# ofsoundof/GRL-Image-Restoration

Measured on NVIDIA H100. Metric: Mpix/s (input pixels) GRL-Base x4 SR 256x256 tiles, higher is better.
Workload: dtype f16

## Files before the change

### grl-image-restoration_b200/csrc/gemm_tc.cu

```cuda
#include <algorithm>

#include "grl_common.cuh"
#include "tc_common.cuh"
#include "ops_tc.h"

namespace grl {
namespace tc {

EncodeTiledFn encode_tiled_fn() {
  static EncodeTiledFn fn = nullptr;
  if (!fn) {
    void* p = nullptr;
    cudaDriverEntryPointQueryResult q;
    if (cudaGetDriverEntryPoint("cuTensorMapEncodeTiled", &p, cudaEnableDefault, &q) == cudaSuccess &&
        q == cudaDriverEntryPointSuccess)
      fn = (EncodeTiledFn)p;
  }
  return fn;
}

__device__ __forceinline__ float gelu_as(float x) {
  const float z = fabsf(x) * 0.70710678118654752440f;
  float t, e;
  asm("rcp.approx.ftz.f32 %0, %1;" : "=f"(t) : "f"(fmaf(0.3275911f, z, 1.0f)));
  asm("ex2.approx.ftz.f32 %0, %1;" : "=f"(e) : "f"(-z * z * 1.4426950408889634f));
  float p = fmaf(1.061405429f, t, -1.453152027f);
  p = fmaf(p, t, 1.421413741f);
  p = fmaf(p, t, -0.284496736f);
  p = fmaf(p, t, 0.254829592f);
  const float erf_abs = fmaf(-p * t, e, 1.0f);
  const float half_x = 0.5f * x;
  return fmaf(half_x, copysignf(erf_abs, x), half_x);
}
__device__ __forceinline__ float tc_act(float v, int act, float slope) {
  if (act == GRL_ACT_GELU) return gelu_as(v);
  if (act == GRL_ACT_LEAKY) return v > 0.f ? v : v * slope;
  return v;
}

constexpr int kStages = 4;
constexpr int kBM = 128, kBK = 64;
constexpr int kTH = 8, kTW = 16;
constexpr int kEpiWarps = 8, kEpiThreads = kEpiWarps * 32, kThreads = kEpiThreads + 32;

__host__ __device__ constexpr int stage_pitch32(int c) { return (c % 8 == 4) ? c : ((c + 3) / 4 * 4 % 8 == 4 ? (c + 3) / 4 * 4 : (c + 3) / 4 * 4 + 4); }

template <int BN>
struct GemmSmem {
  static constexpr int A_BYTES = kBM * kBK * 2;
  static constexpr int B_BYTES = BN * kBK * 2;
  static constexpr int STAGE = A_BYTES + B_BYTES;
  static constexpr int PIPE = kStages * STAGE;
  static constexpr int AP = BN + 4;
  static constexpr int ACC = kBM * AP * 4;
  static constexpr int STG32 = kBM * stage_pitch32(BN <= 192 ? (BN == 192 ? 188 : BN) : 4) * 4;
  static constexpr int STG16 = kBM * (BN + 8) * 2;
  static constexpr int STG = (STG32 > STG16 ? STG32 : STG16);
  static constexpr int OFF_STG = ACC;
  static constexpr int OFF_TOK = ((PIPE > ACC + STG ? PIPE : ACC + STG) + 15) / 16 * 16;
  static constexpr int OFF_PAR = OFF_TOK + 128 * 8 + 128 * 4;
  static constexpr int OFF_MOM = OFF_PAR + 3 * BN * 4;
  static constexpr int OFF_BAR = OFF_MOM + 2 * 128 * 3 * 4;
  static constexpr int TOTAL = OFF_BAR + 128 + 1024 ;
  static_assert(AP % 8 == 4, "accumulator pitch");
  static_assert(TOTAL <= 232448, "shared memory budget");
};

__device__ __forceinline__ void epi_barrier() { asm volatile("bar.sync 1, 256;" ::: "memory"); }

__device__ __forceinline__ void acc_row32(const float* p, uint32_t (&v)[32]) {
#pragma unroll
  for (int j = 0; j < 32; j += 4) {
    const uint4 x = *reinterpret_cast<const uint4*>(p + j);
    v[j] = x.x, v[j + 1] = x.y, v[j + 2] = x.z, v[j + 3] = x.w;
  }
}

template <int BN, int FMT>
__device__ __forceinline__ void mma_loop(float (&acc)[BN / 64][32], uint8_t* smem, uint64_t* full, uint64_t* empty,
                                         int nk_total, int half, int et) {
  using S = GemmSmem<BN>;
  for (int kc = 0; kc < nk_total; ++kc) {
    const int s = kc % kStages;
    mbar_wait(&full[s], (kc / kStages) & 1);
    const uint32_t sa = smem_u32(smem + s * S::STAGE) + half * (64 * 128);
    const uint32_t sb = smem_u32(smem + s * S::STAGE + S::A_BYTES);
    wgmma_fence();
#pragma unroll
    for (int k = 0; k < kBK / 16; ++k) {
      const uint64_t ad = gmma_desc(sa + k * 32, 16, 1024, SWZ_128B);
#pragma unroll
      for (int j = 0; j < BN / 64; ++j) {
        const uint64_t bd = gmma_desc(sb + j * (64 * 128) + k * 32, 16, 1024, SWZ_128B);
        if (FMT == FMT_BF16) wgmma_n64_bf16(acc[j], ad, bd, true);
        else wgmma_n64_f16(acc[j], ad, bd, true);
      }
    }
    wgmma_commit();
    wgmma_wait<1>();
    if (kc > 0 && (et & 127) == 0) mbar_arrive(&empty[(kc - 1) % kStages]);
  }
  wgmma_wait<0>();
}

template <int BN, int EPI, bool CONV>
__global__ void __launch_bounds__(kThreads, 1)
gemm_tc_kernel(const __grid_constant__ CUtensorMap tmA, const __grid_constant__ CUtensorMap tmB, const GemmTcArgs a) {
  extern __shared__ uint8_t smem_raw[];
  uint8_t* smem = reinterpret_cast<uint8_t*>((reinterpret_cast<uintptr_t>(smem_raw) + 1023) & ~uintptr_t(1023));
  using S = GemmSmem<BN>;
  constexpr int AP = S::AP;
  uint64_t* full = reinterpret_cast<uint64_t*>(smem + S::OFF_BAR);
  uint64_t* empty = full + kStages;
  long long* s_tok = reinterpret_cast<long long*>(smem + S::OFF_TOK);
  int* s_img = reinterpret_cast<int*>(smem + S::OFF_TOK + 128 * 8);
  float* s_bias = reinterpret_cast<float*>(smem + S::OFF_PAR);
  float* s_gamma = s_bias + BN;
  float* s_beta = s_gamma + BN;
  float* s_mom = reinterpret_cast<float*>(smem + S::OFF_MOM);
  float* accs = reinterpret_cast<float*>(smem);

  const int warp = threadIdx.x >> 5, lane = threadIdx.x & 31;
  const int n_tiles = a.n_tiles;
  const int m_idx = blockIdx.x / n_tiles;
  const int n0 = (blockIdx.x - m_idx * n_tiles) * BN;
  const int nk_total = a.taps * a.nk;
  int m0 = 0, tb = 0, ty0 = 0, tx0 = 0;
  if (CONV) {
    int t = m_idx;
    const int tx = t % a.tiles_x;
    t /= a.tiles_x;
    const int ty = t % a.tiles_y;
    tb = t / a.tiles_y;
    ty0 = ty * kTH;
    tx0 = tx * kTW;
  } else {
    m0 = m_idx * kBM;
  }

  if (threadIdx.x == 0) {
    for (int s = 0; s < kStages; ++s) {
      mbar_init(&full[s], 1);
      mbar_init(&empty[s], 2);
    }
    mbar_init_fence();
    tma_prefetch_desc(&tmA);
    tma_prefetch_desc(&tmB);
  }
  __syncthreads();

  if (warp == kEpiWarps) {
    if (lane == 0) {
      for (int kc = 0; kc < nk_total; ++kc) {
        const int s = kc % kStages;
        mbar_wait(&empty[s], ((kc / kStages) & 1) ^ 1);
        uint8_t* sa = smem + s * S::STAGE;
        uint8_t* sb = sa + S::A_BYTES;
        mbar_expect_tx(&full[s], S::STAGE);
        if (CONV) {
          const int tap = kc / a.nk, c0 = (kc - tap * a.nk) * kBK;
          tma_load_4d(sa, &tmA, &full[s], c0, tx0 + (tap % 3) - 1, ty0 + (tap / 3) - 1, tb);
        } else {
          tma_load_2d(sa, &tmA, &full[s], kc * kBK, m0);
        }
        tma_load_2d(sb, &tmB, &full[s], kc * kBK, n0);
      }
    }
    return;
  }

  const int et = threadIdx.x;
  const int q = warp & 3;
  const int row = q * 32 + lane;
  const int half = et >> 7;
  const int fmt = a.fmt;
  uint16_t* out16 = reinterpret_cast<uint16_t*>(a.out_bf16);
  {
    long long tok;
    if (CONV) {
      const int y = ty0 + row / kTW, x = tx0 + row % kTW;
      tok = (y < a.H && x < a.W) ? ((long long)tb * a.H + y) * a.W + x : -1;
    } else {
      tok = (long long)m0 + row;
      if (tok >= a.M) tok = -1;
    }
    if (half == 0) {
      s_tok[row] = tok;
      s_img[row] = (EPI == EPI_LN && tok >= 0) ? (int)(tok / a.L) : 0;
    }
    for (int c = et; c < BN; c += kEpiThreads) {
      const int n = n0 + c;
      s_bias[c] = (n < a.N) ? a.bias[n] : 0.f;
      if (EPI == EPI_LN) {
        s_gamma[c] = (c < a.C) ? a.gamma[c] : 0.f;
        s_beta[c] = (c < a.C) ? a.beta[c] : 0.f;
      }
    }
  }
  {
    float acc[BN / 64][32];
#pragma unroll
    for (int j = 0; j < BN / 64; ++j)
#pragma unroll
      for (int e = 0; e < 32; ++e) acc[j][e] = 0.f;
    if (fmt == FMT_BF16) mma_loop<BN, FMT_BF16>(acc, smem, full, empty, nk_total, half, et);
    else mma_loop<BN, FMT_F16>(acc, smem, full, empty, nk_total, half, et);
    epi_barrier();
    const int w = (et >> 5) & 3, r0 = half * 64 + 16 * w + (lane >> 2), cq = 2 * (lane & 3);
#pragma unroll
    for (int j = 0; j < BN / 64; ++j)
#pragma unroll
      for (int i = 0; i < 8; ++i) {
        const int c = j * 64 + 8 * i + cq;
        *reinterpret_cast<float2*>(accs + r0 * AP + c) = make_float2(acc[j][4 * i], acc[j][4 * i + 1]);
        *reinterpret_cast<float2*>(accs + (r0 + 8) * AP + c) = make_float2(acc[j][4 * i + 2], acc[j][4 * i + 3]);
      }
  }
  epi_barrier();
  uint32_t v[32];

    if (EPI == EPI_BIAS_ACT && a.epi_mode == 2) {
      const long long tok = s_tok[row];
      for (int c0 = 32 * half; c0 < BN; c0 += 64) {
        if (n0 + c0 >= a.N) break;
        acc_row32(accs + row * AP + c0, v);
        if (tok < 0) continue;
        float o[32];
#pragma unroll
        for (int j = 0; j < 32; ++j) {
          const int n = n0 + c0 + j;
          float val = tc_act(__uint_as_float(v[j]) + s_bias[c0 + j], a.act, a.slope);
          if (a.res_f32 && n < a.N_f32) val += __ldg(a.res_f32 + tok * a.ldr + n);
          o[j] = (n < a.N) ? val : 0.f;
          if (a.out_f32 && n < a.N_f32) a.out_f32[tok * a.ldo_f32 + n] = o[j];
          if (CONV && a.out_nchw && n < a.N_f32) {
            const int r = a.nchw_r, rr = r * r;
            const int c = n / rr, q = n - c * rr;
            const int yy = (ty0 + row / kTW) * r + q / r, xx = (tx0 + row % kTW) * r + q % r;
            if (yy < a.Hc && xx < a.Wc)
              a.out_nchw[(((long long)tb * (a.N_f32 / rr) + c) * a.Hc + yy) * a.Wc + xx] = fmaf(o[j], a.post_scale, a.post_shift[c & 3]);
          }
        }
        if (out16) {
#pragma unroll
          for (int j = 0; j < 32; j += 8)
            if (n0 + c0 + j < a.ldo_bf16)
              *reinterpret_cast<uint4*>(out16 + tok * a.ldo_bf16 + n0 + c0 + j) =
                  make_uint4(pack16(o[j], o[j + 1], fmt), pack16(o[j + 2], o[j + 3], fmt), pack16(o[j + 4], o[j + 5], fmt),
                             pack16(o[j + 6], o[j + 7], fmt));
        }
      }
    } else if (a.epi_mode == 1) {
      const int Cw = (EPI == EPI_LN) ? a.C : a.N_f32;
      const int pitch = stage_pitch32(Cw);
      float* stg = reinterpret_cast<float*>(smem + S::OFF_STG);
      const bool res_in_stage = a.res_f32 != nullptr;
      if (res_in_stage) {
        const int C4r = Cw >> 2, ewr = et >> 5;
        for (int r = ewr; r < kBM; r += kEpiWarps) {
          const long long rtok = s_tok[r];
          for (int c4 = lane; c4 < C4r; c4 += 32)
            cp_async_16(stg + r * pitch + c4 * 4, a.res_f32 + (rtok >= 0 ? rtok : 0) * a.ldr + c4 * 4, rtok >= 0);
        }
        cp_async_commit();
      }
      if (EPI == EPI_LN) {
        float s1 = 0.f, s2 = 0.f, x0 = 0.f;
        int nh = 0;
        for (int c0 = 32 * half; c0 < Cw; c0 += 64) {
          acc_row32(accs + row * AP + c0, v);
          if (c0 == 32 * half) x0 = __uint_as_float(v[0]) + s_bias[c0];
#pragma unroll
          for (int j = 0; j < 32; ++j)
            if (c0 + j < Cw) {
              const float d = __uint_as_float(v[j]) + s_bias[c0 + j] - x0;
              s1 += d;
              s2 = fmaf(d, d, s2);
              ++nh;
            }
        }
        {
          const float fn = (float)nh;
          const float m1 = nh > 0 ? s1 / fn : 0.f;
          s_mom[(half * kBM + row) * 3 + 0] = x0 + m1;
          s_mom[(half * kBM + row) * 3 + 1] = nh > 0 ? fmaxf(s2 - s1 * m1, 0.f) : 0.f;
          s_mom[(half * kBM + row) * 3 + 2] = fn;
        }
        if (res_in_stage) cp_async_wait<0>();
        epi_barrier();
        float mean, rstd;
        {
          const float m0 = s_mom[row * 3 + 0], q0 = s_mom[row * 3 + 1], c0n = s_mom[row * 3 + 2];
          const float m1 = s_mom[(kBM + row) * 3 + 0], q1 = s_mom[(kBM + row) * 3 + 1], c1n = s_mom[(kBM + row) * 3 + 2];
          const float n = c0n + c1n, d = (c1n > 0.f) ? m1 - m0 : 0.f;
          mean = m0 + d * (c1n / n);
          const float M2 = q0 + q1 + d * d * (c0n * c1n / n);
          rstd = rsqrtf(M2 / n + a.eps);
        }
        for (int c0 = 32 * half; c0 < Cw; c0 += 64) {
          acc_row32(accs + row * AP + c0, v);
#pragma unroll
          for (int j = 0; j < 32; j += 4) {
            if (c0 + j < Cw) {
              float4* sp = reinterpret_cast<float4*>(stg + row * pitch + c0 + j);
              float4 acc4 = res_in_stage ? *sp : make_float4(0.f, 0.f, 0.f, 0.f);
              float o4[4] = {acc4.x, acc4.y, acc4.z, acc4.w};
#pragma unroll
              for (int e = 0; e < 4; ++e) {
                const int c = c0 + j + e;
                o4[e] += ((__uint_as_float(v[j + e]) + s_bias[c] - mean) * rstd * s_gamma[c] + s_beta[c]) * a.res_scale;
              }
              *sp = make_float4(o4[0], o4[1], o4[2], o4[3]);
            }
          }
        }
      } else {
        if (res_in_stage) {
          cp_async_wait<0>();
          epi_barrier();
        }
        for (int c0 = 32 * half; c0 < Cw; c0 += 64) {
          acc_row32(accs + row * AP + c0, v);
#pragma unroll
          for (int j = 0; j < 32; j += 4) {
            if (c0 + j < Cw) {
              float4* sp = reinterpret_cast<float4*>(stg + row * pitch + c0 + j);
              float4 acc4 = res_in_stage ? *sp : make_float4(0.f, 0.f, 0.f, 0.f);
              float o4[4] = {acc4.x, acc4.y, acc4.z, acc4.w};
#pragma unroll
              for (int e = 0; e < 4; ++e) o4[e] += tc_act(__uint_as_float(v[j + e]) + s_bias[c0 + j + e], a.act, a.slope);
              *sp = make_float4(o4[0], o4[1], o4[2], o4[3]);
            }
          }
        }
      }
      epi_barrier();
      const int C4 = Cw >> 2;
      const int P4 = out16 ? (int)(a.ldo_bf16 >> 2) : C4;
      const int ew = et >> 5;
      const bool has_cab = (EPI == EPI_LN) && a.cab_y != nullptr;
      const uint16_t* caby = reinterpret_cast<const uint16_t*>(a.cab_y);
      constexpr int RB = 8;
      for (int cbase = 0; cbase < P4; cbase += 32) {
        const int c4 = cbase + lane;
        const bool col_real = c4 < C4, col_any = c4 < P4;
        for (int rb = 0; rb < kBM / kEpiWarps; rb += RB) {
          long long tok[RB];
          float4 gg[RB];
          uint2 cy[RB];
#pragma unroll
          for (int i = 0; i < RB; ++i) {
            tok[i] = s_tok[ew + kEpiWarps * (rb + i)];
            gg[i] = make_float4(0.f, 0.f, 0.f, 0.f);
            cy[i] = make_uint2(0u, 0u);
            if (tok[i] >= 0 && col_real) {
              if (has_cab) {
                cy[i] = __ldg(reinterpret_cast<const uint2*>(caby + tok[i] * a.ld_caby + c4 * 4));
                gg[i] = __ldg(reinterpret_cast<const float4*>(a.cab_gate + (long long)s_img[ew + kEpiWarps * (rb + i)] * Cw + c4 * 4));
              }
            }
          }
#pragma unroll
          for (int i = 0; i < RB; ++i) {
            if (tok[i] < 0 || !col_any) continue;
            float4 val = make_float4(0.f, 0.f, 0.f, 0.f);
            if (col_real) {
              val = *reinterpret_cast<const float4*>(stg + (ew + kEpiWarps * (rb + i)) * pitch + c4 * 4);
              if (has_cab) {
                const float2 c01 = unpack16(cy[i].x, fmt), c23 = unpack16(cy[i].y, fmt);
                val.x = fmaf(c01.x, gg[i].x, val.x), val.y = fmaf(c01.y, gg[i].y, val.y);
                val.z = fmaf(c23.x, gg[i].z, val.z), val.w = fmaf(c23.y, gg[i].w, val.w);
              }
              if (a.out_f32) *reinterpret_cast<float4*>(a.out_f32 + tok[i] * a.ldo_f32 + c4 * 4) = val;
            }
            if (out16)
              *reinterpret_cast<uint2*>(out16 + tok[i] * a.ldo_bf16 + c4 * 4) =
                  make_uint2(pack16(val.x, val.y, fmt), pack16(val.z, val.w, fmt));
          }
        }
      }
    } else {
      constexpr int P16 = BN + 8;
      uint16_t* stg = reinterpret_cast<uint16_t*>(smem + S::OFF_STG);
      const int ncols = min(BN, a.N - n0);
      for (int c0 = 32 * half; c0 < ncols; c0 += 64) {
        acc_row32(accs + row * AP + c0, v);
        float o[32];
        if (EPI == EPI_QKV) {
          const int slot = (n0 + c0) >> 5;
          float ss = 0.f;
#pragma unroll
          for (int j = 0; j < 32; ++j) {
            o[j] = __uint_as_float(v[j]) + s_bias[c0 + j];
            ss = fmaf(o[j], o[j], ss);
          }
          const float sc = __ldg(a.slot_scale + slot);
          const float mul = sc > 0.f ? sc * rsqrtf(fmaxf(ss, 1e-24f)) : 1.0f;
#pragma unroll
          for (int j = 0; j < 32; ++j) o[j] *= mul;
        } else {
#pragma unroll
          for (int j = 0; j < 32; ++j) o[j] = tc_act(__uint_as_float(v[j]) + s_bias[c0 + j], a.act, a.slope);
        }
#pragma unroll
        for (int j = 0; j < 32; j += 8)
          *reinterpret_cast<uint4*>(stg + row * P16 + c0 + j) =
              make_uint4(pack16(o[j], o[j + 1], fmt), pack16(o[j + 2], o[j + 3], fmt), pack16(o[j + 4], o[j + 5], fmt),
                         pack16(o[j + 6], o[j + 7], fmt));
      }
      epi_barrier();
      const int nvec = min((long long)ncols, a.ldo_bf16 - n0) >> 3;
      const int ew = et >> 5;
      if (CONV && a.ps_r > 0) {
        const int ps = a.ps_r, Cq = a.N / (ps * ps);
        const int nv = min(BN, a.N - n0) >> 3;
#pragma unroll 4
        for (int r = ew; r < kBM; r += kEpiWarps) {
          if (s_tok[r] < 0) continue;
          const int y = ty0 + r / kTW, x = tx0 + r % kTW;
          for (int vv = lane; vv < nv; vv += 32) {
            const int n = n0 + vv * 8;
            const int q = n / Cq, c = n - q * Cq;
            const long long dtok = ((long long)tb * a.H * ps + y * ps + q / ps) * ((long long)a.W * ps) + x * ps + q % ps;
            *reinterpret_cast<uint4*>(out16 + dtok * a.ldo_bf16 + c) = *reinterpret_cast<const uint4*>(stg + r * P16 + vv * 8);
          }
        }
      } else {
#pragma unroll 4
        for (int r = ew; r < kBM; r += kEpiWarps) {
          const long long tok = s_tok[r];
          if (tok < 0) continue;
          for (int vv = lane; vv < nvec; vv += 32)
            *reinterpret_cast<uint4*>(out16 + tok * a.ldo_bf16 + n0 + vv * 8) = *reinterpret_cast<const uint4*>(stg + r * P16 + vv * 8);
        }
      }
    }

}

static int make_map(CUtensorMap* m, const void* base, int rank, const cuuint64_t* dims, const cuuint64_t* strides_bytes,
                    const cuuint32_t* box, int fmt) {
  EncodeTiledFn fn = encode_tiled_fn();
  if (!fn) return fail(GRL_ERR_CUDA, "cuTensorMapEncodeTiled is not available from the driver");
  cuuint32_t ones[5] = {1, 1, 1, 1, 1};
  CUresult rc = fn(m, fmt == FMT_BF16 ? CU_TENSOR_MAP_DATA_TYPE_BFLOAT16 : CU_TENSOR_MAP_DATA_TYPE_FLOAT16, (cuuint32_t)rank, const_cast<void*>(base), dims, strides_bytes,
                   box, ones, CU_TENSOR_MAP_INTERLEAVE_NONE, CU_TENSOR_MAP_SWIZZLE_128B,
                   CU_TENSOR_MAP_L2_PROMOTION_L2_128B, CU_TENSOR_MAP_FLOAT_OOB_FILL_NONE);
  if (rc != CUDA_SUCCESS) return fail(GRL_ERR_CUDA, "cuTensorMapEncodeTiled failed with CUresult %d", (int)rc);
  return GRL_OK;
}

template <int BN, int EPI, bool CONV>
static int launch_one(const CUtensorMap& tmA, const CUtensorMap& tmB, const GemmTcArgs& a, dim3 grid, cudaStream_t st) {
  auto kern = gemm_tc_kernel<BN, EPI, CONV>;
  static bool configured[kMaxDevices] = {false};
  int dev = 0;
  GRL_CUDA(cudaGetDevice(&dev));
  if (dev < 0 || dev >= kMaxDevices || !configured[dev]) {
    GRL_CUDA(cudaFuncSetAttribute(kern, cudaFuncAttributeMaxDynamicSharedMemorySize, GemmSmem<BN>::TOTAL));
    if (dev >= 0 && dev < kMaxDevices) configured[dev] = true;
  }
  kern<<<grid, kThreads, GemmSmem<BN>::TOTAL, st>>>(tmA, tmB, a);
  GRL_LAUNCH_CHECK("gemm_tc_kernel");
  return GRL_OK;
}

template <int EPI, bool CONV>
static int dispatch_bn(int bn, const CUtensorMap& tmA, const CUtensorMap& tmB, const GemmTcArgs& a, dim3 grid,
                       cudaStream_t st) {
  switch (bn) {
    case 64: return launch_one<64, EPI, CONV>(tmA, tmB, a, grid, st);
    case 128: return launch_one<128, EPI, CONV>(tmA, tmB, a, grid, st);
    case 192: return launch_one<192, EPI, CONV>(tmA, tmB, a, grid, st);
    case 256: return launch_one<256, EPI, CONV>(tmA, tmB, a, grid, st);
  }
  return fail(GRL_ERR_INVALID, "gemm_tc: unsupported tile width %d", bn);
}

int pick_bn(int npad) {
  if (npad <= 64) return 64;
  if (npad <= 128) return 128;
  if (npad % 192 == 0 || npad <= 192) return 192;
  if (npad % 256 == 0) return 256;
  return npad % 128 == 0 ? 128 : 192;
}

int plan_gemm_tc(const GemmTcProblem& p, GemmTcArgs& a, int* bn_out) {
  GRL_REQUIRE(p.kpad % kBK == 0 && p.kpad > 0, "gemm_tc: K pad %d must be a multiple of 64", p.kpad);
  GRL_REQUIRE(p.npad % 32 == 0 && p.npad > 0, "gemm_tc: N pad %d must be a multiple of 32", p.npad);
  int bn = (p.epi == EPI_LN) ? (p.npad <= 64 ? 64 : p.npad <= 128 ? 128 : p.npad <= 192 ? 192 : 256) : pick_bn(p.npad);
  GRL_REQUIRE(p.epi != EPI_LN || p.npad <= 256, "gemm_tc: LayerNorm epilogue needs the whole row in one tile (N=%d)",
              p.npad);
  const bool conv = p.taps == 9;
  if (a.ps_r > 0)
    GRL_REQUIRE(conv && p.epi == EPI_BIAS_ACT && !a.out_f32 && !a.res_f32 && a.out_bf16 && a.N % (a.ps_r * a.ps_r) == 0 &&
                    (a.N / (a.ps_r * a.ps_r)) % 8 == 0 && a.ldo_bf16 >= a.N / (a.ps_r * a.ps_r),
                "gemm_tc: pixel-shuffle store needs a 16-bit-only conv epilogue with N %% r^2 == 0 and N / r^2 %% 8 == 0");
  if (a.out_nchw)
    GRL_REQUIRE(conv && p.epi == EPI_BIAS_ACT && a.nchw_r >= 1 && a.N_f32 % (a.nchw_r * a.nchw_r) == 0 &&
                    a.N_f32 / (a.nchw_r * a.nchw_r) <= 4 && a.Hc > 0 && a.Wc > 0,
                "gemm_tc: NCHW tail store needs a conv with <= 4 output channels");
  GRL_REQUIRE(p.taps == 1 || p.taps == 9, "gemm_tc: taps must be 1 or 9");
  a.epi_mode = 0;
  if (p.epi == EPI_LN || (p.epi == EPI_BIAS_ACT && (a.out_f32 || a.res_f32))) {
    const int cw = p.epi == EPI_LN ? a.C : a.N_f32;
    const int cap = bn == 64 ? GemmSmem<64>::STG : bn == 128 ? GemmSmem<128>::STG : bn == 192 ? GemmSmem<192>::STG
                                                                                               : GemmSmem<256>::STG;
    const bool ok = p.npad <= bn && cw > 0 && cw % 4 == 0 && kBM * stage_pitch32(cw) * 4 <= cap &&
                    (!a.out_f32 || a.ldo_f32 % 4 == 0) && (!a.res_f32 || a.ldr % 4 == 0) &&
                    (!a.out_bf16 || a.ldo_bf16 % 4 == 0);
    GRL_REQUIRE(ok || p.epi != EPI_LN, "gemm_tc: LayerNorm epilogue needs C %% 4 == 0 and C <= 188 (got %d)", cw);
    a.epi_mode = ok ? 1 : 2;
  }
  if (a.out_nchw) a.epi_mode = 2;
  GRL_REQUIRE(p.epi == EPI_BIAS_ACT || p.epi == EPI_QKV || p.epi == EPI_LN, "gemm_tc: unknown epilogue %d", p.epi);
  GRL_REQUIRE(!conv || p.epi == EPI_BIAS_ACT, "gemm_tc: %s epilogue is linear-only", p.epi == EPI_QKV ? "QKV" : "LN");
  a.nk = p.kpad / kBK;
  a.taps = p.taps;
  a.n_tiles = ceil_div(p.npad, bn);
  if (conv) {
    a.H = p.H, a.W = p.W;
    a.tiles_x = ceil_div(p.W, kTW), a.tiles_y = ceil_div(p.H, kTH);
    a.M = (long long)p.B * p.H * p.W;
    GRL_REQUIRE((long long)a.tiles_x * a.tiles_y * p.B * a.n_tiles < (1ll << 31), "gemm_tc: grid too large");
    a.total_tiles = a.tiles_x * a.tiles_y * p.B * a.n_tiles;
  } else {
    a.M = p.M;
    GRL_REQUIRE((long long)ceil_div(p.M, kBM) * a.n_tiles < (1ll << 31), "gemm_tc: grid too large");
    a.total_tiles = (int)(ceil_div(p.M, kBM) * a.n_tiles);
  }
  *bn_out = bn;
  return GRL_OK;
}

int launch_gemm_tc(const GemmTcProblem& p, GemmTcArgs a, cudaStream_t st) {
  int bn = 0, rc;
  if ((rc = plan_gemm_tc(p, a, &bn)) != GRL_OK) return rc;
  if (a.M == 0) return GRL_OK;
  CUtensorMap tmA, tmB;
  if (p.taps == 9) {
    cuuint64_t dims[4] = {(cuuint64_t)p.kpad, (cuuint64_t)p.W, (cuuint64_t)p.H, (cuuint64_t)p.B};
    cuuint64_t str[3] = {(cuuint64_t)p.kpad * 2, (cuuint64_t)p.W * p.kpad * 2, (cuuint64_t)p.H * p.W * p.kpad * 2};
    cuuint32_t box[4] = {(cuuint32_t)kBK, (cuuint32_t)kTW, (cuuint32_t)kTH, 1};
    if ((rc = make_map(&tmA, p.x, 4, dims, str, box, a.fmt)) != GRL_OK) return rc;
  } else {
    cuuint64_t dims[2] = {(cuuint64_t)p.kpad, (cuuint64_t)p.M};
    cuuint64_t str[1] = {(cuuint64_t)p.kpad * 2};
    cuuint32_t box[2] = {(cuuint32_t)kBK, (cuuint32_t)kBM};
    if ((rc = make_map(&tmA, p.x, 2, dims, str, box, a.fmt)) != GRL_OK) return rc;
  }
  {
    cuuint64_t dims[2] = {(cuuint64_t)p.kpad * p.taps, (cuuint64_t)p.npad};
    cuuint64_t str[1] = {(cuuint64_t)p.kpad * p.taps * 2};
    cuuint32_t box[2] = {(cuuint32_t)kBK, (cuuint32_t)bn};
    if ((rc = make_map(&tmB, p.w, 2, dims, str, box, a.fmt)) != GRL_OK) return rc;
  }
  const dim3 grid((unsigned)a.total_tiles);
  switch (p.epi) {
    case EPI_QKV: return dispatch_bn<EPI_QKV, false>(bn, tmA, tmB, a, grid, st);
    case EPI_LN: return dispatch_bn<EPI_LN, false>(bn, tmA, tmB, a, grid, st);
  }
  return p.taps == 9 ? dispatch_bn<EPI_BIAS_ACT, true>(bn, tmA, tmB, a, grid, st)
                     : dispatch_bn<EPI_BIAS_ACT, false>(bn, tmA, tmB, a, grid, st);
}

}
}
```

Measured before the change: 1.575.

## Add persistent warp-specialized TMA/WGMMA GEMM kernel with cross-tile producer pipelining

Adds a persistent GEMM kernel launched with at most one CTA per SM that loops over output tiles. A producer warp keeps issuing TMA loads through the mbarrier ring across tile boundaries, so loads for the next tile can overlap the epilogue of the current one, and bias staging is reused when n0 repeats. Dispatch routes BN 128/192/256 bias-act and QKV GEMMs (and 3x3 convs) to it when epi_mode is 0. The risks are fewer pipeline stages because the smem budget also has to hold the epilogue tile, and tail imbalance from static tile striding.

New measurement: 1.627 (median of 6 runs). 3.3% higher.

```diff
diff --git a/grl-image-restoration_b200/csrc/gemm_tc.cu b/grl-image-restoration_b200/csrc/gemm_tc.cu
--- a/grl-image-restoration_b200/csrc/gemm_tc.cu
+++ b/grl-image-restoration_b200/csrc/gemm_tc.cu
@@ -438,6 +438,244 @@
 
 }
 
+template <int BN, int EPI>
+struct PersistSmem {
+  static constexpr int STAGE = GemmSmem<BN>::STAGE;
+  static constexpr int TILE = EPI == EPI_QKV ? kBM * (BN + 4) * 4 : kBM * (BN + 8) * 2;
+  static constexpr int TABLES = 128 * 8 + BN * 4 + 2 * kStages * 8;
+  static constexpr int AVAIL = 232448 - 1024  - TABLES - TILE;
+  static constexpr int ST = AVAIL / STAGE < kStages ? AVAIL / STAGE : kStages;
+  static constexpr int OFF_TILE = ST * STAGE;
+  static constexpr int OFF_TOK = OFF_TILE + TILE;
+  static constexpr int OFF_BIAS = OFF_TOK + 128 * 8;
+  static constexpr int OFF_BAR = OFF_BIAS + BN * 4;
+  static constexpr int TOTAL = OFF_BAR + 2 * kStages * 8 + 1024;
+  static_assert(ST >= 2 && TOTAL <= 232448, "shared memory budget");
+};
+
+struct TileAt {
+  int n0, m0, tb, ty0, tx0;
+};
+template <int BN, bool CONV>
+__device__ __forceinline__ TileAt tile_at(const GemmTcArgs& a, int t) {
+  TileAt r = {0, 0, 0, 0, 0};
+  const int m_idx = t / a.n_tiles;
+  r.n0 = (t - m_idx * a.n_tiles) * BN;
+  if (CONV) {
+    int u = m_idx;
+    const int tx = u % a.tiles_x;
+    u /= a.tiles_x;
+    const int ty = u % a.tiles_y;
+    r.tb = u / a.tiles_y;
+    r.ty0 = ty * kTH;
+    r.tx0 = tx * kTW;
+  } else {
+    r.m0 = m_idx * kBM;
+  }
+  return r;
+}
+
+template <int BN, int FMT, int ST>
+__device__ __forceinline__ void mma_loop_ring(float (&acc)[BN / 64][32], uint8_t* smem, uint64_t* full, uint64_t* empty,
+                                              int nk_total, int half, int et, int& s, uint32_t& ph) {
+  using S = GemmSmem<BN>;
+  int prev = 0;
+  for (int kc = 0; kc < nk_total; ++kc) {
+    mbar_wait(&full[s], ph);
+    const uint32_t sa = smem_u32(smem + s * S::STAGE) + half * (64 * 128);
+    const uint32_t sb = smem_u32(smem + s * S::STAGE + S::A_BYTES);
+    wgmma_fence();
+#pragma unroll
+    for (int k = 0; k < kBK / 16; ++k) {
+      const uint64_t ad = gmma_desc(sa + k * 32, 16, 1024, SWZ_128B);
+#pragma unroll
+      for (int j = 0; j < BN / 64; ++j) {
+        const uint64_t bd = gmma_desc(sb + j * (64 * 128) + k * 32, 16, 1024, SWZ_128B);
+        if (FMT == FMT_BF16) wgmma_n64_bf16(acc[j], ad, bd, true);
+        else wgmma_n64_f16(acc[j], ad, bd, true);
+      }
+    }
+    wgmma_commit();
+    wgmma_wait<1>();
+    if (kc > 0 && (et & 127) == 0) mbar_arrive(&empty[prev]);
+    prev = s;
+    if (++s == ST) s = 0, ph ^= 1;
+  }
+  wgmma_wait<0>();
+  if ((et & 127) == 0) mbar_arrive(&empty[prev]);
+}
+
+template <int BN, int EPI, bool CONV>
+__global__ void __launch_bounds__(kThreads, 1)
+gemm_tc_persistent_kernel(const __grid_constant__ CUtensorMap tmA, const __grid_constant__ CUtensorMap tmB,
+                          const GemmTcArgs a) {
+  static_assert(EPI == EPI_BIAS_ACT || EPI == EPI_QKV, "16-bit-only epilogues");
+  extern __shared__ uint8_t smem_raw[];
+  uint8_t* smem = reinterpret_cast<uint8_t*>((reinterpret_cast<uintptr_t>(smem_raw) + 1023) & ~uintptr_t(1023));
+  using S = PersistSmem<BN, EPI>;
+  constexpr int ST = S::ST, AP = BN + 4, P16 = BN + 8;
+  uint64_t* full = reinterpret_cast<uint64_t*>(smem + S::OFF_BAR);
+  uint64_t* empty = full + kStages;
+  long long* s_tok = reinterpret_cast<long long*>(smem + S::OFF_TOK);
+  float* s_bias = reinterpret_cast<float*>(smem + S::OFF_BIAS);
+  float* accs = reinterpret_cast<float*>(smem + S::OFF_TILE);
+  uint16_t* stg16 = reinterpret_cast<uint16_t*>(smem + S::OFF_TILE);
+  const int warp = threadIdx.x >> 5, lane = threadIdx.x & 31;
+  const int nk_total = a.taps * a.nk;
+
+  if (threadIdx.x == 0) {
+    for (int s = 0; s < ST; ++s) {
+      mbar_init(&full[s], 1);
+      mbar_init(&empty[s], 2);
+    }
+    mbar_init_fence();
+    tma_prefetch_desc(&tmA);
+    tma_prefetch_desc(&tmB);
+  }
+  __syncthreads();
+
+  if (warp == kEpiWarps) {
+    if (lane == 0) {
+      int s = 0;
+      uint32_t ph = 0;
+      for (int t = blockIdx.x; t < a.total_tiles; t += gridDim.x) {
+        const TileAt tl = tile_at<BN, CONV>(a, t);
+        for (int kc = 0; kc < nk_total; ++kc) {
+          mbar_wait(&empty[s], ph ^ 1);
+          uint8_t* sa = smem + s * S::STAGE;
+          uint8_t* sb = sa + GemmSmem<BN>::A_BYTES;
+          mbar_expect_tx(&full[s], S::STAGE);
+          if (CONV) {
+            const int tap = kc / a.nk, c0 = (kc - tap * a.nk) * kBK;
+            tma_load_4d(sa, &tmA, &full[s], c0, tl.tx0 + (tap % 3) - 1, tl.ty0 + (tap / 3) - 1, tl.tb);
+          } else {
+            tma_load_2d(sa, &tmA, &full[s], kc * kBK, tl.m0);
+          }
+          tma_load_2d(sb, &tmB, &full[s], kc * kBK, tl.n0);
+          if (++s == ST) s = 0, ph ^= 1;
+        }
+      }
+    }
+    return;
+  }
+
+  const int et = threadIdx.x;
+  const int row = (warp & 3) * 32 + lane;
+  const int half = et >> 7;
+  const int fmt = a.fmt;
+  uint16_t* out16 = reinterpret_cast<uint16_t*>(a.out_bf16);
+  int s = 0, staged_n0 = -1;
+  uint32_t ph = 0;
+  for (int t = blockIdx.x; t < a.total_tiles; t += gridDim.x) {
+    const TileAt tl = tile_at<BN, CONV>(a, t);
+    const int n0 = tl.n0;
+    float acc[BN / 64][32];
+#pragma unroll
+    for (int j = 0; j < BN / 64; ++j)
+#pragma unroll
+      for (int e = 0; e < 32; ++e) acc[j][e] = 0.f;
+    if (fmt == FMT_BF16) mma_loop_ring<BN, FMT_BF16, ST>(acc, smem, full, empty, nk_total, half, et, s, ph);
+    else mma_loop_ring<BN, FMT_F16, ST>(acc, smem, full, empty, nk_total, half, et, s, ph);
+    epi_barrier();
+    {
+      long long tok;
+      if (CONV) {
+        const int y = tl.ty0 + row / kTW, x = tl.tx0 + row % kTW;
+        tok = (y < a.H && x < a.W) ? ((long long)tl.tb * a.H + y) * a.W + x : -1;
+      } else {
+        tok = (long long)tl.m0 + row;
+        if (tok >= a.M) tok = -1;
+      }
+      if (half == 0) s_tok[row] = tok;
+    }
+    const bool restage = n0 != staged_n0;
+    if (restage) {
+      for (int c = et; c < BN; c += kEpiThreads) s_bias[c] = (n0 + c < a.N) ? a.bias[n0 + c] : 0.f;
+      staged_n0 = n0;
+    }
+    const int w = (et >> 5) & 3, r0 = half * 64 + 16 * w + (lane >> 2), cq = 2 * (lane & 3);
+    if constexpr (EPI == EPI_BIAS_ACT) {
+      if (restage) epi_barrier();
+#pragma unroll
+      for (int j = 0; j < BN / 64; ++j)
+#pragma unroll
+        for (int i = 0; i < 8; ++i) {
+          const int c = j * 64 + 8 * i + cq;
+          const float b0 = s_bias[c], b1 = s_bias[c + 1];
+          *reinterpret_cast<uint32_t*>(stg16 + r0 * P16 + c) =
+              pack16(tc_act(acc[j][4 * i] + b0, a.act, a.slope), tc_act(acc[j][4 * i + 1] + b1, a.act, a.slope), fmt);
+          *reinterpret_cast<uint32_t*>(stg16 + (r0 + 8) * P16 + c) =
+              pack16(tc_act(acc[j][4 * i + 2] + b0, a.act, a.slope), tc_act(acc[j][4 * i + 3] + b1, a.act, a.slope), fmt);
+        }
+    } else {
+#pragma unroll
+      for (int j = 0; j < BN / 64; ++j)
+#pragma unroll
+        for (int i = 0; i < 8; ++i) {
+          const int c = j * 64 + 8 * i + cq;
+          *reinterpret_cast<float2*>(accs + r0 * AP + c) = make_float2(acc[j][4 * i], acc[j][4 * i + 1]);
+          *reinterpret_cast<float2*>(accs + (r0 + 8) * AP + c) = make_float2(acc[j][4 * i + 2], acc[j][4 * i + 3]);
+        }
+    }
+    epi_barrier();
+    const int ncols = min(BN, a.N - n0);
+    if constexpr (EPI == EPI_QKV) {
+      uint32_t v[32];
+      for (int c0 = 32 * half; c0 < ncols; c0 += 64) {
+        acc_row32(accs + row * AP + c0, v);
+        float o[32];
+        const int slot = (n0 + c0) >> 5;
+        float ss = 0.f;
+#pragma unroll
+        for (int j = 0; j < 32; ++j) {
+          o[j] = __uint_as_float(v[j]) + s_bias[c0 + j];
+          ss = fmaf(o[j], o[j], ss);
+        }
+        const float sc = __ldg(a.slot_scale + slot);
+        const float mul = sc > 0.f ? sc * rsqrtf(fmaxf(ss, 1e-24f)) : 1.0f;
+#pragma unroll
+        for (int j = 0; j < 32; ++j) o[j] *= mul;
+        uint16_t* dst = reinterpret_cast<uint16_t*>(accs + row * AP + c0);
+#pragma unroll
+        for (int j = 0; j < 32; j += 8)
+          *reinterpret_cast<uint4*>(dst + j) =
+              make_uint4(pack16(o[j], o[j + 1], fmt), pack16(o[j + 2], o[j + 3], fmt), pack16(o[j + 4], o[j + 5], fmt),
+                         pack16(o[j + 6], o[j + 7], fmt));
+      }
+      epi_barrier();
+    }
+    auto src16 = [&](int r, int vv) -> const uint4* {
+      if constexpr (EPI == EPI_QKV) return reinterpret_cast<const uint4*>(accs + r * AP + (vv >> 2) * 32) + (vv & 3);
+      else return reinterpret_cast<const uint4*>(stg16 + r * P16 + vv * 8);
+    };
+    const int ew = et >> 5;
+    if (CONV && a.ps_r > 0) {
+      const int ps = a.ps_r, Cq = a.N / (ps * ps);
+      const int nv = ncols >> 3;
+#pragma unroll 4
+      for (int r = ew; r < kBM; r += kEpiWarps) {
+        if (s_tok[r] < 0) continue;
+        const int y = tl.ty0 + r / kTW, x = tl.tx0 + r % kTW;
+        for (int vv = lane; vv < nv; vv += 32) {
+          const int n = n0 + vv * 8;
+          const int q = n / Cq, c = n - q * Cq;
+          const long long dtok = ((long long)tl.tb * a.H * ps + y * ps + q / ps) * ((long long)a.W * ps) + x * ps + q % ps;
+          *reinterpret_cast<uint4*>(out16 + dtok * a.ldo_bf16 + c) = *src16(r, vv);
+        }
+      }
+    } else {
+      const int nvec = min((long long)ncols, a.ldo_bf16 - n0) >> 3;
+#pragma unroll 4
+      for (int r = ew; r < kBM; r += kEpiWarps) {
+        const long long tok = s_tok[r];
+        if (tok < 0) continue;
+        for (int vv = lane; vv < nvec; vv += 32)
+          *reinterpret_cast<uint4*>(out16 + tok * a.ldo_bf16 + n0 + vv * 8) = *src16(r, vv);
+      }
+    }
+  }
+}
+
 static int make_map(CUtensorMap* m, const void* base, int rank, const cuuint64_t* dims, const cuuint64_t* strides_bytes,
                     const cuuint32_t* box, int fmt) {
   EncodeTiledFn fn = encode_tiled_fn();
@@ -462,6 +700,24 @@
   }
   kern<<<grid, kThreads, GemmSmem<BN>::TOTAL, st>>>(tmA, tmB, a);
   GRL_LAUNCH_CHECK("gemm_tc_kernel");
+  return GRL_OK;
+}
+
+template <int BN, int EPI, bool CONV>
+static int launch_persistent(const CUtensorMap& tmA, const CUtensorMap& tmB, const GemmTcArgs& a, cudaStream_t st) {
+  auto kern = gemm_tc_persistent_kernel<BN, EPI, CONV>;
+  constexpr int smem = PersistSmem<BN, EPI>::TOTAL;
+  static int sms[kMaxDevices] = {0};
+  int dev = 0;
+  GRL_CUDA(cudaGetDevice(&dev));
+  int n_sm = (dev >= 0 && dev < kMaxDevices) ? sms[dev] : 0;
+  if (n_sm == 0) {
+    GRL_CUDA(cudaFuncSetAttribute(kern, cudaFuncAttributeMaxDynamicSharedMemorySize, smem));
+    GRL_CUDA(cudaDeviceGetAttribute(&n_sm, cudaDevAttrMultiProcessorCount, dev));
+    if (dev >= 0 && dev < kMaxDevices) sms[dev] = n_sm;
+  }
+  kern<<<std::min(a.total_tiles, n_sm), kThreads, smem, st>>>(tmA, tmB, a);
+  GRL_LAUNCH_CHECK("gemm_tc_persistent_kernel");
   return GRL_OK;
 }
 
@@ -555,6 +811,17 @@
     cuuint32_t box[2] = {(cuuint32_t)kBK, (cuuint32_t)bn};
     if ((rc = make_map(&tmB, p.w, 2, dims, str, box, a.fmt)) != GRL_OK) return rc;
   }
+  if (a.epi_mode == 0 && (bn == 128 || bn == 192 || (bn == 256 && p.epi == EPI_BIAS_ACT))) {
+    if (p.epi == EPI_QKV) return bn == 128 ? launch_persistent<128, EPI_QKV, false>(tmA, tmB, a, st)
+                                           : launch_persistent<192, EPI_QKV, false>(tmA, tmB, a, st);
+    if (p.taps == 9)
+      return bn == 128 ? launch_persistent<128, EPI_BIAS_ACT, true>(tmA, tmB, a, st)
+             : bn == 192 ? launch_persistent<192, EPI_BIAS_ACT, true>(tmA, tmB, a, st)
+                         : launch_persistent<256, EPI_BIAS_ACT, true>(tmA, tmB, a, st);
+    return bn == 128 ? launch_persistent<128, EPI_BIAS_ACT, false>(tmA, tmB, a, st)
+           : bn == 192 ? launch_persistent<192, EPI_BIAS_ACT, false>(tmA, tmB, a, st)
+                       : launch_persistent<256, EPI_BIAS_ACT, false>(tmA, tmB, a, st);
+  }
   const dim3 grid((unsigned)a.total_tiles);
   switch (p.epi) {
     case EPI_QKV: return dispatch_bn<EPI_QKV, false>(bn, tmA, tmB, a, grid, st);
```
